# jgsimard/big-dreamer

Hardware: AMD Instinct MI355X
Metric: latent transitions/sec (RSSM + imagination) at batch=50 chunk=50 H=15 (higher is better)
Workload: dtype f32

## Files before the change

big_dreamer_amd/csrc/observe_ksplit.hip:

```cpp
#include "bd_cluster.h"

namespace bd {

#ifdef BD_STAMPS
__device__ unsigned long long g_kstamps[64];
#define BD_KSTAMP(slot)                                                                                  \
    do {                                                                                                 \
        if (blockIdx.x == 0 && threadIdx.x == 0 && t == 5) g_kstamps[slot] = __builtin_amdgcn_s_memtime(); \
    } while (0)
#else
#define BD_KSTAMP(slot)
#endif

constexpr int kKsMaxS = 4;
constexpr int kKsMaxA = 2;

__device__ __forceinline__ void ks_store4(float* p, floatx4 v) {
    asm volatile("s_nop 7\n\ts_nop 3\n\tglobal_store_dwordx4 %0, %1, off sc1\n\ts_nop 1" ::"v"(p), "v"(v) : "memory");
}
__device__ __forceinline__ floatx4 ks_load4(const float* p) {
    const unsigned long long lo = ld_sc1_u64(p), hi = ld_sc1_u64(p + 2);
    return floatx4{__uint_as_float((unsigned)lo), __uint_as_float((unsigned)(lo >> 32)), __uint_as_float((unsigned)hi),
                   __uint_as_float((unsigned)(hi >> 32))};
}

__device__ __forceinline__ void ks_emit(float* img, int lane, floatx4 v) { ks_store4(img + lane * 4, v); }

constexpr int kKsChunk = 8;

__device__ __forceinline__ floatx4 ks_reduce(const float* base, size_t src_stride, int first, int stride, int C, int lane) {
    floatx4 s = floatx4{0.f, 0.f, 0.f, 0.f};
    const float* p = base + lane * 4;
    for (int m0 = first; m0 < C; m0 += kKsChunk * stride) {
        floatx4 v[kKsChunk];
#pragma unroll
        for (int i = 0; i < kKsChunk; ++i) {
            const int src = m0 + i * stride;
            v[i] = floatx4{0.f, 0.f, 0.f, 0.f};
            if (src < C) v[i] = ks_load4(p + (size_t)src * src_stride);
        }
#pragma unroll
        for (int i = 0; i < kKsChunk; ++i) s += v[i];
    }
    return s;
}
__device__ __forceinline__ void ks_handoff(unsigned* flags, int c, int C, unsigned epoch, unsigned* err, unsigned limit,
                                           unsigned code) {
    publish(flags + c, epoch);
    wait_all(flags, C, epoch, err, limit, code);
}
__device__ __forceinline__ floatx4 mfma4(floatx4 a, floatx4 b, floatx4 acc) {
#pragma unroll
    for (int j = 0; j < 4; ++j) acc = mfma16(a[j], b[j], acc);
    return acc;
}
__device__ __forceinline__ void ks_settle(floatx4& v) { asm volatile("" : "+v"(v)); }
template <int N>
__device__ __forceinline__ void ks_settle(floatx4 (&v)[N]) {
#pragma unroll
    for (int i = 0; i < N; ++i) ks_settle(v[i]);
}
#define KS_SETTLE_BEGIN() asm volatile("s_waitcnt vmcnt(0)" ::: "memory")

__device__ __forceinline__ floatx4 ks_frag(const float* w, int nb, int Kb, int kb, int lane, bool ok) {
    return ok ? reinterpret_cast<const floatx4*>(w)[((size_t)nb * Kb + kb) * 64 + lane] : floatx4{0.f, 0.f, 0.f, 0.f};
}

__device__ __forceinline__ floatx4 mfmaT(floatx4 w, floatx4 x, floatx4 acc) {
#pragma unroll
    for (int j = 0; j < 4; ++j) acc = mfma16(w[j], x[j], acc);
    return acc;
}
__device__ __forceinline__ floatx4 ks_row4(const float* p, int n_valid) {
    floatx4 v = floatx4{0.f, 0.f, 0.f, 0.f};
    if (n_valid >= 4) {
        __builtin_memcpy(&v, p, 16);
        return v;
    }
#pragma unroll
    for (int i = 0; i < 4; ++i)
        if (i < n_valid) v[i] = p[i];
    return v;
}
__device__ __forceinline__ void ks_put4(float* p, floatx4 v, int n_valid) {
    if (n_valid >= 4) {
        __builtin_memcpy(p, &v, 16);
        return;
    }
#pragma unroll
    for (int i = 0; i < 4; ++i)
        if (i < n_valid) p[i] = v[i];
}

__global__ __launch_bounds__(kThreads) void observe_kfwd_ns_kernel(bd_observe_fwd_args a_, float* __restrict__ ws, int C, int tiles,
                                                                   unsigned spin_limit) {
    extern __shared__ __attribute__((aligned(16))) float smem[];
    BD_KARGS(bd_observe_fwd_args, ap);
#define a (*ap)
    const ScanDims d(a.Be, a.S, a.A, a.Hd);
    const int Kb_h = d.Kb_h, Kb_s = d.Kb_s, Kb_a = d.Kb_a, Kb_hd = d.Kb_hd;
    const int tile = blockIdx.x / C, c = blockIdx.x - tile * C;
    const int row0 = tile * 16, F = a.Be + a.S, Np = Kb_s * 16;
    const int lane = threadIdx.x & 63;
    const int wave = __builtin_amdgcn_readfirstlane((int)(threadIdx.x >> 6));
    const KsplitFwdLds L(d, a.S);
    float* sf = smem + L.sf;
    float* af = smem + L.af;
    float* red = smem + L.red;
    float* plain = smem + L.plain;
    float* xf = smem + L.xf;
    float* hf = smem + L.hf;
    float* gpart = smem + L.gpart;

    unsigned* flags = reinterpret_cast<unsigned*>(ws) + tile * kMaxCluster;
    unsigned* err = reinterpret_cast<unsigned*>(ws) + tiles * kMaxCluster;
    const KsBuf kb_(C);
    float* xbase = ws + cluster_ws_header_floats(tiles) + (size_t)tile * kKsCopies * kb_.total;

    floatx4 we_s[2][kKsMaxS], we_a[2][kKsMaxA], be4x[2];
    floatx4 wg[2][6], wq[2];
#pragma unroll
    for (int i = 0; i < 2; ++i) {
        const int nbo = wave + kWaves * i;
        const bool ok = nbo < Kb_h;
#pragma unroll
        for (int kb = 0; kb < kKsMaxS; ++kb) we_s[i][kb] = ks_frag(a.w_embed_s, nbo, Kb_s, kb, lane, ok && kb < Kb_s);
#pragma unroll
        for (int kb = 0; kb < kKsMaxA; ++kb) we_a[i][kb] = ks_frag(a.w_embed_a, nbo, Kb_a, kb, lane, ok && kb < Kb_a);
#pragma unroll
        for (int j = 0; j < 4; ++j) {
            const int col = nbo * 16 + 4 * (lane >> 4) + j;
            be4x[i][j] = (ok && col < a.Be) ? a.b_embed[col] : 0.f;
        }
        wg[i][0] = ks_frag(a.w_ir, c, Kb_h, nbo, lane, ok); wg[i][1] = ks_frag(a.w_iz, c, Kb_h, nbo, lane, ok);
        wg[i][2] = ks_frag(a.w_in, c, Kb_h, nbo, lane, ok); wg[i][3] = ks_frag(a.w_hr, c, Kb_h, nbo, lane, ok);
        wg[i][4] = ks_frag(a.w_hz, c, Kb_h, nbo, lane, ok); wg[i][5] = ks_frag(a.w_hn, c, Kb_h, nbo, lane, ok);
        wq[i] = ks_frag(a.w_q1h, nbo, Kb_h, c, lane, nbo < Kb_hd);
    }
    const int npairs = 2 * Kb_s, nparts = kWaves / npairs;
    const int pair = wave % npairs, part = wave / npairs;
    const int pair_nb = pair >> 1, pair_raw = pair & 1;
    const bool has_pair = part == 0, sums_pair = part < nparts;
    floatx4 wh = ks_frag(pair_raw ? a.w_q2s : a.w_q2m, pair_nb, Kb_hd, c, lane, has_pair && c < Kb_hd);
    const int frow = lane & 15, fcol0 = c * 16 + 4 * (lane >> 4);
    const int grow = row0 + frow;
    const int nbe = a.Be - fcol0 < 0 ? 0 : (a.Be - fcol0 < 4 ? a.Be - fcol0 : 4);
    const int nhd = a.Hd - fcol0 < 0 ? 0 : (a.Hd - fcol0 < 4 ? a.Hd - fcol0 : 4);
    const bool rok = grow < a.B;
    floatx4 br4 = floatx4{0.f, 0.f, 0.f, 0.f}, bz4 = br4, bni4 = br4, bnh4 = br4, bq4 = br4;
#pragma unroll
    for (int i = 0; i < 4; ++i) {
        if (i < nbe) {
            const int col = fcol0 + i;
            br4[i] = a.b_ih[col] + a.b_hh[col];
            bz4[i] = a.b_ih[a.Be + col] + a.b_hh[a.Be + col];
            bni4[i] = a.b_ih[2 * a.Be + col];
            bnh4[i] = a.b_hh[2 * a.Be + col];
        }
        if (i < nhd) bq4[i] = a.b_q1[fcol0 + i];
    }
    floatx4 bh4 = floatx4{0.f, 0.f, 0.f, 0.f};
    if (has_pair) {
#pragma unroll
        for (int i = 0; i < 4; ++i) {
            const int col = pair_nb * 16 + 4 * (lane >> 4) + i;
            if (col < a.S) bh4[i] = a.b_q2[pair_raw * a.S + col];
        }
    }
    floatx4 h4 = rok ? ks_row4(a.init_belief + (size_t)grow * a.Be + fcol0, nbe) : floatx4{0.f, 0.f, 0.f, 0.f};
    floatx4* __restrict__ XF4 = reinterpret_cast<floatx4*>(xf);
    floatx4* __restrict__ HF4 = reinterpret_cast<floatx4*>(hf);
#pragma unroll
    for (int i = 0; i < 2; ++i) {
        const int nbo = wave + kWaves * i;
        if (nbo < Kb_h) {
            const int col0 = nbo * 16 + 4 * (lane >> 4);
            const int nv = a.Be - col0 < 0 ? 0 : (a.Be - col0 < 4 ? a.Be - col0 : 4);
            HF4[nbo * 64 + lane] = rok ? ks_row4(a.init_belief + (size_t)grow * a.Be + col0, nv) : floatx4{0.f, 0.f, 0.f, 0.f};
        }
    }
    for (int i = threadIdx.x; i < 16 * Kb_s * 16; i += blockDim.x) {
        const int r = i / (Kb_s * 16), k = i - r * (Kb_s * 16);
        float v = 0.f;
        if (row0 + r < a.B && k < a.S) {
            v = a.init_state[(size_t)(row0 + r) * a.S + k] * (a.nonterm ? a.nonterm[row0 + r] : 1.f);
            if (c == 0 && a.sv_s) a.sv_s[(size_t)(row0 + r) * a.S + k] = v;
        }
        sf[frag_idx(r, k)] = v;
    }
    for (int i = threadIdx.x; i < 16 * Kb_a * 16; i += blockDim.x) {
        const int r = i / (Kb_a * 16), k = i - r * (Kb_a * 16);
        af[frag_idx(r, k)] = (row0 + r < a.B && k < a.A) ? a.actions[(size_t)(row0 + r) * a.A + k] : 0.f;
    }
    lds_barrier();

    KS_SETTLE_BEGIN();
    ks_settle(we_s[0]); ks_settle(we_s[1]); ks_settle(we_a[0]); ks_settle(we_a[1]); ks_settle(be4x);
    ks_settle(wg[0]); ks_settle(wg[1]); ks_settle(wq);
    ks_settle(wh);
    ks_settle(br4); ks_settle(bz4); ks_settle(bni4); ks_settle(bnh4); ks_settle(bq4); ks_settle(bh4); ks_settle(h4);
    const bool lead = (c == 0);
    floatx4* __restrict__ RED4 = reinterpret_cast<floatx4*>(red);
    floatx4* __restrict__ REDB = RED4 + kWaves * 64;
    floatx4* __restrict__ GP4 = reinterpret_cast<floatx4*>(gpart);
    const floatx4 z4 = floatx4{0.f, 0.f, 0.f, 0.f};

    auto load_nt = [&](int t, int e) {
        const int r = e / a.S;
        return (a.nonterm && t < a.T && e < 16 * a.S && row0 + r < a.B) ? a.nonterm[(size_t)t * a.B + row0 + r] : 1.f;
    };
    auto load_ac = [&](int t, int i) {
        const int r = i / (Kb_a * 16), k = i - r * (Kb_a * 16);
        return (t < a.T && i < 16 * Kb_a * 16 && row0 + r < a.B && k < a.A) ? a.actions[((size_t)t * a.B + row0 + r) * a.A + k] : 0.f;
    };

    for (int t = 0; t < a.T; ++t) {
        const size_t tb = (size_t)t * a.B;
        const int tid = bd_tid();
        float* xb = xbase + (size_t)(t & 1) * kb_.total;
        float* hx = xb + kb_.g;
        BD_KSTAMP(0);
        BD_KARGS_FRESH(ap);
        BD_KSTAMP(1);
        {
            const floatx4* __restrict__ S4 = reinterpret_cast<const floatx4*>(sf) + lane;
            const floatx4* __restrict__ A4 = reinterpret_cast<const floatx4*>(af) + lane;
#pragma unroll
            for (int i = 0; i < 2; ++i) {
                const int nbo = wave + kWaves * i;
                if (nbo < Kb_h) {
                    floatx4 acc = be4x[i];
#pragma unroll
                    for (int kb = 0; kb < kKsMaxS; ++kb)
                        if (kb < Kb_s) acc = mfmaT(we_s[i][kb], S4[kb * 64], acc);
#pragma unroll
                    for (int kb = 0; kb < kKsMaxA; ++kb)
                        if (kb < Kb_a) acc = mfmaT(we_a[i][kb], A4[kb * 64], acc);
                    floatx4 x4;
                    const int col0 = nbo * 16 + 4 * (lane >> 4);
#pragma unroll
                    for (int j = 0; j < 4; ++j) x4[j] = (rok && col0 + j < a.Be) ? elu(acc[j]) : 0.f;
                    XF4[nbo * 64 + lane] = x4;
                    if (nbo == c && rok && a.sv_x) ks_put4(a.sv_x + (tb + grow) * a.Be + fcol0, x4, nbe);
                }
            }
        }
        lds_barrier();
        BD_KSTAMP(2);
        BD_KARGS_FRESH(ap);
        {
            floatx4 R = z4, Z = z4, NI = z4, NH = z4;
#pragma unroll
            for (int i = 0; i < 2; ++i) {
                const int kb = wave + kWaves * i;
                if (kb < Kb_h) {
                    const floatx4 xk = XF4[kb * 64 + lane], hk = HF4[kb * 64 + lane];
                    R = mfmaT(wg[i][0], xk, R); Z = mfmaT(wg[i][1], xk, Z); NI = mfmaT(wg[i][2], xk, NI);
                    R = mfmaT(wg[i][3], hk, R); Z = mfmaT(wg[i][4], hk, Z); NH = mfmaT(wg[i][5], hk, NH);
                }
            }
            GP4[(wave * 4 + 0) * 64 + lane] = R; GP4[(wave * 4 + 1) * 64 + lane] = Z;
            GP4[(wave * 4 + 2) * 64 + lane] = NI; GP4[(wave * 4 + 3) * 64 + lane] = NH;
        }
        lds_barrier();
        BD_KSTAMP(3);
        BD_KSTAMP(4);
        {
            const int g = wave & 3, half = wave >> 2;
            floatx4 s4 = z4;
#pragma unroll
            for (int w = 0; w < 4; ++w) s4 += GP4[((half * 4 + w) * 4 + g) * 64 + lane];
            RED4[wave * 64 + lane] = s4;
        }
        lds_barrier();
        {
            const floatx4 R = RED4[0 * 64 + lane] + RED4[4 * 64 + lane] + br4, Z = RED4[1 * 64 + lane] + RED4[5 * 64 + lane] + bz4;
            const floatx4 NI = RED4[2 * 64 + lane] + RED4[6 * 64 + lane] + bni4, NH = RED4[3 * 64 + lane] + RED4[7 * 64 + lane] + bnh4;
            floatx4 rr4, zz4, nn4;
#pragma unroll
            for (int i = 0; i < 4; ++i) {
                rr4[i] = sigmoidf(R[i]);
                zz4[i] = sigmoidf(Z[i]);
                nn4[i] = tanh_act(NI[i] + rr4[i] * NH[i]);
                h4[i] = (rok && i < nbe) ? (1.f - zz4[i]) * nn4[i] + zz4[i] * h4[i] : 0.f;
            }
            if (wave == 0) {
                ks_store4(hx + (size_t)c * 256 + lane * 4, h4);
                if (rok) {
                    ks_put4(a.feat + (tb + grow) * F + fcol0, h4, nbe);
                    if (a.sv_gates) {
                        float* gg = a.sv_gates + (tb + grow) * 4 * a.Be + fcol0;
                        ks_put4(gg, rr4, nbe); ks_put4(gg + a.Be, zz4, nbe); ks_put4(gg + 2 * a.Be, nn4, nbe); ks_put4(gg + 3 * a.Be, NH, nbe);
                    }
                }
            }
        }
        BD_KSTAMP(5);
        BD_KARGS_FRESH(ap);
        const float n_nt = load_nt(t + 1, tid), n_ac = load_ac(t + 1, tid);
        const floatx4 pre4 = rok ? ks_row4(a.pre_emb + (tb + grow) * a.Hd + fcol0, nhd) : z4;
        float eps = 0.f;
        {
            const int row = tid / a.S, col = tid - row * a.S;
            if (tid < 16 * a.S && row0 + row < a.B) eps = a.eps_post[(tb + row0 + row) * a.S + col];
        }
#pragma unroll
        for (int i = 0; i < 2; ++i) {
            const int nbo = wave + kWaves * i;
            if (nbo < Kb_hd) ks_emit(xb + kb_.q + (size_t)(nbo * C + c) * kKsImg, lane, mfmaT(wq[i], h4, z4));
        }
        BD_KSTAMP(6);
        ks_handoff(flags, c, C, (unsigned)(3 * t + 2), err, spin_limit, kErrFwd);
        BD_KSTAMP(7);
        REDB[wave * 64 + lane] = c < Kb_hd ? ks_reduce(xb + kb_.q + (size_t)(c * C) * kKsImg, kKsImg, wave, kWaves, C, lane) : z4;
#pragma unroll
        for (int i = 0; i < 2; ++i) {
            const int nbo = wave + kWaves * i;
            if (nbo < Kb_h) HF4[nbo * 64 + lane] = ks_load4(hx + (size_t)nbo * 256 + lane * 4);
        }
        lds_barrier();
        floatx4 q4 = bq4 + pre4;
        for (int w = 0; w < kWaves; ++w) q4 += REDB[w * 64 + lane];
#pragma unroll
        for (int i = 0; i < 4; ++i) q4[i] = (rok && i < nhd) ? elu(q4[i]) : 0.f;
        if (wave == 0 && rok && a.sv_q) ks_put4(a.sv_q + (tb + grow) * a.Hd + fcol0, q4, nhd);
        BD_KSTAMP(8);
        BD_KARGS_FRESH(ap);
        if (has_pair) ks_emit(xb + kb_.s + (size_t)(c * 8 + pair) * kKsImg, lane, mfmaT(wh, q4, z4));
        BD_KSTAMP(9);
        ks_handoff(flags, c, C, (unsigned)(3 * t + 3), err, spin_limit, kErrFwd);
        BD_KSTAMP(10);
        BD_KARGS_FRESH(ap);
        if (sums_pair) {
            floatx4 v = ks_reduce(xb + kb_.s + (size_t)pair * kKsImg, (size_t)8 * kKsImg, part, nparts, C, lane);
            if (part == 0) v += bh4;
            float* pl = plain + (size_t)part * 2 * 16 * Np;
#pragma unroll
            for (int i = 0; i < 4; ++i) pl[pair_raw * 16 * Np + frow * Np + pair_nb * 16 + 4 * (lane >> 4) + i] = v[i];
        }
        lds_barrier();
        if (tid < 16 * a.S) {
            const int e = tid;
            const int row = e / a.S, col = e - row * a.S;
            const int gr = row0 + row;
            float st = 0.f;
            if (gr < a.B) {
                float Mn = plain[row * Np + col], Rw = plain[16 * Np + row * Np + col];
                for (int pt = 1; pt < nparts; ++pt) {
                    Mn += plain[pt * 2 * 16 * Np + row * Np + col];
                    Rw += plain[pt * 2 * 16 * Np + 16 * Np + row * Np + col];
                }
                const float ee = eps;
                const float sd = softplusf(Rw) + a.min_std;
                st = Mn + sd * ee;
                if (lead) {
                    const size_t ix = (tb + gr) * a.S + col;
                    a.post_mean[ix] = Mn;
                    a.post_std[ix] = sd;
                    a.feat[(tb + gr) * F + a.Be + col] = st;
                }
            }
            const float mv = st * n_nt;
            sf[frag_idx(row, col)] = mv;
            if (lead && a.sv_s && t + 1 < a.T && gr < a.B) a.sv_s[(tb + a.B + gr) * a.S + col] = mv;
        }
        if (tid < 16 * Kb_a * 16) af[frag_idx(tid / (Kb_a * 16), tid % (Kb_a * 16))] = n_ac;
        lds_barrier();
        BD_KSTAMP(11);
    }
#undef a
}

__global__ __launch_bounds__(kThreads) void observe_kbwd_kernel(bd_observe_bwd_args a_, float* __restrict__ ws, int C, int tiles,
                                                                unsigned spin_limit) {
    extern __shared__ __attribute__((aligned(16))) float smem[];
    BD_KARGS(bd_observe_bwd_args, ap);
#define a (*ap)
    const ScanDims d(a.Be, a.S, a.A, a.Hd);
    const int Kb_h = d.Kb_h, Kb_s = d.Kb_s, Kb_hd = d.Kb_hd;
    const int tile = blockIdx.x / C, c = blockIdx.x - tile * C;
    const int row0 = tile * 16, F = a.Be + a.S;
    const int lane = threadIdx.x & 63;
    const int wave = __builtin_amdgcn_readfirstlane((int)(threadIdx.x >> 6));
    const KsplitBwdLds L(d, a.S);
    float* dM = smem + L.dM;
    float* dRaw = smem + L.dRaw;
    float* ds_plain = smem + L.ds_plain;
    const int nparts = L.nparts;
    const int dsp_stride = L.dsp_stride;
    float* red = smem + L.red;

    unsigned* flags = reinterpret_cast<unsigned*>(ws) + tile * kMaxCluster;
    unsigned* err = reinterpret_cast<unsigned*>(ws) + tiles * kMaxCluster;
    const KsBuf kb_(C);
    float* xbase = ws + cluster_ws_header_floats(tiles) + (size_t)tile * kKsCopies * kb_.total;

    floatx4 w2m[kKsMaxS], w2s[kKsMaxS];
#pragma unroll
    for (int kb = 0; kb < kKsMaxS; ++kb) {
        w2m[kb] = ks_frag(a.wt_q2m, c, Kb_s, kb, lane, kb < Kb_s && c < Kb_hd);
        w2s[kb] = ks_frag(a.wt_q2s, c, Kb_s, kb, lane, kb < Kb_s && c < Kb_hd);
    }
    floatx4 w1[2], wg[2][6];
#pragma unroll
    for (int i = 0; i < 2; ++i) {
        const int nbo = wave + kWaves * i;
        const bool ok = nbo < Kb_h;
        w1[i] = ks_frag(a.wt_q1h, nbo, Kb_hd, c, lane, ok && c < Kb_hd);
        wg[i][0] = ks_frag(a.wt_ir, nbo, Kb_h, c, lane, ok); wg[i][1] = ks_frag(a.wt_iz, nbo, Kb_h, c, lane, ok);
        wg[i][2] = ks_frag(a.wt_in, nbo, Kb_h, c, lane, ok); wg[i][3] = ks_frag(a.wt_hr, nbo, Kb_h, c, lane, ok);
        wg[i][4] = ks_frag(a.wt_hz, nbo, Kb_h, c, lane, ok); wg[i][5] = ks_frag(a.wt_hn, nbo, Kb_h, c, lane, ok);
    }
    const int sblk = wave % Kb_s, spart = wave / Kb_s;
    floatx4 wes = ks_frag(a.wt_embed_s, sblk, Kb_h, c, lane, spart == 0);
    const int frow = lane & 15, fcol0 = c * 16 + 4 * (lane >> 4);
    const int grow = row0 + frow;
    const int nbe = a.Be - fcol0 < 0 ? 0 : (a.Be - fcol0 < 4 ? a.Be - fcol0 : 4);
    const int nhd = a.Hd - fcol0 < 0 ? 0 : (a.Hd - fcol0 < 4 ? a.Hd - fcol0 : 4);
    const bool rok = grow < a.B;

    for (int i = threadIdx.x; i < nparts * dsp_stride; i += blockDim.x) ds_plain[i] = 0.f;
    lds_barrier();

    KS_SETTLE_BEGIN();
    ks_settle(w2m); ks_settle(w2s); ks_settle(w1); ks_settle(wg[0]); ks_settle(wg[1]);
    ks_settle(wes);
    const bool lead = (c == 0);
    floatx4* __restrict__ RED4 = reinterpret_cast<floatx4*>(red);
    floatx4* __restrict__ REDB = RED4 + kWaves * 64;
    const floatx4 z4 = floatx4{0.f, 0.f, 0.f, 0.f};
    floatx4 dhc4 = z4;
    unsigned epoch = 0;

    struct B1v { float dfs, dpm, eps, dps, pstd; };
    struct Svv { floatx4 svq4, svx4, gr4, gz4, gn4, gh4, hp4, dft4; };
    auto load_b1 = [&](int t, int i) {
        B1v v{0.f, 0.f, 0.f, 0.f, 0.f};
        const int r = i / (Kb_s * 16), k = i - r * (Kb_s * 16);
        const int gr = row0 + r;
        if (i < 16 * Kb_s * 16 && gr < a.B && k < a.S) {
            const size_t tb = (size_t)t * a.B, idx = (tb + gr) * a.S + k;
            v.dfs = a.dfeat[(tb + gr) * F + a.Be + k];
            v.dpm = a.dpost_mean ? a.dpost_mean[idx] : 0.f;
            v.eps = a.eps_post[idx];
            v.dps = a.dpost_std ? a.dpost_std[idx] : 0.f;
            v.pstd = a.post_std[idx];
        }
        return v;
    };
    auto load_sv = [&](int t) {
        Svv v;
        v.svq4 = floatx4{1.f, 1.f, 1.f, 1.f};
        v.svx4 = v.svq4;
        v.gr4 = v.gz4 = v.gn4 = v.gh4 = v.hp4 = v.dft4 = z4;
        if (rok) {
            const size_t tb = (size_t)t * a.B;
            v.svq4 = ks_row4(a.sv_q + (tb + grow) * a.Hd + fcol0, nhd);
            v.svx4 = ks_row4(a.sv_x + (tb + grow) * a.Be + fcol0, nbe);
            const float* gg = a.sv_gates + (tb + grow) * 4 * a.Be + fcol0;
            v.gr4 = ks_row4(gg, nbe); v.gz4 = ks_row4(gg + a.Be, nbe); v.gn4 = ks_row4(gg + 2 * a.Be, nbe); v.gh4 = ks_row4(gg + 3 * a.Be, nbe);
            v.hp4 = t > 0 ? ks_row4(a.feat + (tb - a.B + grow) * F + fcol0, nbe) : ks_row4(a.init_belief + (size_t)grow * a.Be + fcol0, nbe);
            v.dft4 = ks_row4(a.dfeat + (tb + grow) * F + fcol0, nbe);
        }
        return v;
    };
    B1v nb1{0.f, 0.f, 0.f, 0.f, 0.f};
    Svv nsv{z4, z4, z4, z4, z4, z4, z4, z4};
    nb1 = load_b1(a.T - 1, (int)threadIdx.x);
    nsv = load_sv(a.T - 1);

    for (int t = a.T - 1; t >= 0; --t) {
        const size_t tb = (size_t)t * a.B;
        const int tid = bd_tid();
        float* xb = xbase + (size_t)(t & 1) * kb_.total;
        BD_KSTAMP(16);
        BD_KARGS_FRESH(ap);
        const B1v cb1 = nb1;
        const Svv sv = nsv;
        if (t > 0) {
            nb1 = load_b1(t - 1, tid);
            nsv = load_sv(t - 1);
        }
        if (tid < 16 * Kb_s * 16) {
            const int i = tid;
            const int r = i / (Kb_s * 16), k = i - r * (Kb_s * 16);
            const int gr = row0 + r;
            float dm = 0.f, dr = 0.f;
            if (gr < a.B && k < a.S) {
                const B1v v = cb1;
                float dst = v.dfs;
                for (int pt = 0; pt < nparts; ++pt) dst += ds_plain[pt * dsp_stride + r * a.S + k];
                dm = dst + v.dpm;
                const float dsd = dst * v.eps + v.dps;
                dr = dsd * one_minus_exp_neg(v.pstd - a.min_std);
                if (lead) {
                    a.d_q2_out[(tb + gr) * 2 * a.S + k] = dm;
                    a.d_q2_out[(tb + gr) * 2 * a.S + a.S + k] = dr;
                }
            }
            dM[frag_idx(r, k)] = dm;
            dRaw[frag_idx(r, k)] = dr;
        }
        const floatx4 svq4 = sv.svq4, svx4 = sv.svx4, gr4 = sv.gr4, gz4 = sv.gz4, gn4 = sv.gn4, gh4 = sv.gh4, hp4 = sv.hp4, dft4 = sv.dft4;
        lds_barrier();
        BD_KSTAMP(17);
        floatx4 dq4;
        {
            floatx4 acc = z4;
            const floatx4* __restrict__ M4 = reinterpret_cast<const floatx4*>(dM) + lane;
            const floatx4* __restrict__ R4 = reinterpret_cast<const floatx4*>(dRaw) + lane;
#pragma unroll
            for (int kb = 0; kb < kKsMaxS; ++kb)
                if (kb < Kb_s) {
                    acc = mfmaT(w2m[kb], M4[kb * 64], acc);
                    acc = mfmaT(w2s[kb], R4[kb * 64], acc);
                }
#pragma unroll
            for (int i = 0; i < 4; ++i) dq4[i] = (rok && i < nhd) ? acc[i] * elu_grad_from_out(svq4[i]) : 0.f;
            if (wave == 0 && rok) ks_put4(a.d_q1_pre + (tb + grow) * a.Hd + fcol0, dq4, nhd);
        }
        BD_KSTAMP(18);
        BD_KARGS_FRESH(ap);
        ++epoch;
#pragma unroll
        for (int i = 0; i < 2; ++i) {
            const int nbo = wave + kWaves * i;
            if (nbo < Kb_h) ks_emit(xb + kb_.q + (size_t)(nbo * C + c) * kKsImg, lane, mfmaT(w1[i], dq4, z4));
        }
        BD_KSTAMP(19);
        ks_handoff(flags, c, C, epoch, err, spin_limit, kErrBwd);
        BD_KSTAMP(20);
        RED4[wave * 64 + lane] = ks_reduce(xb + kb_.q + (size_t)(c * C) * kKsImg, kKsImg, wave, kWaves, C, lane);
        lds_barrier();
        floatx4 vr4, vz4, vni4, vnh4, carry4;
        {
            floatx4 dh4 = dhc4 + dft4;
            for (int w = 0; w < kWaves; ++w) dh4 += RED4[w * 64 + lane];
#pragma unroll
            for (int i = 0; i < 4; ++i) {
                const bool ok = rok && i < nbe;
                const float dh = ok ? dh4[i] : 0.f;
                const float rr = gr4[i], zz = gz4[i], nn = gn4[i], hn = gh4[i];
                const float dn = dh * (1.f - zz);
                const float dz = dh * (hp4[i] - nn);
                vni4[i] = dn * (1.f - nn * nn);
                vnh4[i] = vni4[i] * rr;
                vr4[i] = vni4[i] * hn * rr * (1.f - rr);
                vz4[i] = dz * zz * (1.f - zz);
                carry4[i] = dh * zz;
            }
            if (wave == 0 && rok) {
                float* gi = a.d_gi + (tb + grow) * 3 * a.Be + fcol0;
                float* ghh = a.d_gh + (tb + grow) * 3 * a.Be + fcol0;
                ks_put4(gi, vr4, nbe); ks_put4(gi + a.Be, vz4, nbe); ks_put4(gi + 2 * a.Be, vni4, nbe);
                ks_put4(ghh, vr4, nbe); ks_put4(ghh + a.Be, vz4, nbe); ks_put4(ghh + 2 * a.Be, vnh4, nbe);
            }
        }
        BD_KSTAMP(21);
        BD_KARGS_FRESH(ap);
        ++epoch;
#pragma unroll
        for (int i = 0; i < 2; ++i) {
            const int nbo = wave + kWaves * i;
            if (nbo < Kb_h) {
                floatx4 DX = mfmaT(wg[i][0], vr4, z4), DH = mfmaT(wg[i][3], vr4, z4);
                DX = mfmaT(wg[i][1], vz4, DX); DH = mfmaT(wg[i][4], vz4, DH);
                DX = mfmaT(wg[i][2], vni4, DX); DH = mfmaT(wg[i][5], vnh4, DH);
                float* dst = xb + kb_.g + ((size_t)(nbo * C + c) * 2) * kKsImg;
                ks_emit(dst, lane, DX); ks_emit(dst + kKsImg, lane, DH);
            }
        }
        BD_KSTAMP(22);
        ks_handoff(flags, c, C, epoch, err, spin_limit, kErrBwd);
        BD_KSTAMP(23);
        {
            const int g = wave & 1, quarter = wave >> 1;
            REDB[wave * 64 + lane] = ks_reduce(xb + kb_.g + ((size_t)(c * C) * 2 + g) * kKsImg, (size_t)2 * kKsImg, quarter, 4, C, lane);
        }
        lds_barrier();
        floatx4 de4;
        {
            floatx4 DX = z4, DH = z4;
            for (int qd = 0; qd < 4; ++qd) { DX += REDB[(2 * qd) * 64 + lane]; DH += REDB[(2 * qd + 1) * 64 + lane]; }
#pragma unroll
            for (int i = 0; i < 4; ++i) {
                const bool ok = rok && i < nbe;
                de4[i] = ok ? DX[i] * elu_grad_from_out(svx4[i]) : 0.f;
                dhc4[i] = ok ? carry4[i] + DH[i] : 0.f;
            }
            if (wave == 0 && rok) ks_put4(a.d_embed_pre + (tb + grow) * a.Be + fcol0, de4, nbe);
        }
        BD_KSTAMP(24);
        BD_KARGS_FRESH(ap);
        ++epoch;
        if (spart == 0) ks_emit(xb + kb_.s + (size_t)(c * 8 + sblk) * kKsImg, lane, mfmaT(wes, de4, z4));
        BD_KSTAMP(25);
        ks_handoff(flags, c, C, epoch, err, spin_limit, kErrBwd);
        BD_KSTAMP(26);
        BD_KARGS_FRESH(ap);
        if (spart < nparts) {
            const floatx4 v = ks_reduce(xb + kb_.s + (size_t)sblk * kKsImg, (size_t)8 * kKsImg, spart, nparts, C, lane);
            const float mk = rok ? (a.nonterm ? a.nonterm[tb + grow] : 1.f) : 0.f;
#pragma unroll
            for (int i = 0; i < 4; ++i) {
                const int col = sblk * 16 + 4 * (lane >> 4) + i;
                if (col < a.S) ds_plain[spart * dsp_stride + frow * a.S + col] = v[i] * mk;
            }
        }
        lds_barrier();
        BD_KSTAMP(27);
    }
#undef a
}

int& ksplit_mode() {
    static int m = -1;
    return m;
}

bool ksplit_ok(int Be, int S, int A, int Hd, int C) {
    if (ksplit_mode() == 0) return false;
    return C == cdiv(Be, 16) && C <= 2 * kWaves && cdiv(Hd, 16) <= C && cdiv(S, 16) <= kKsMaxS && cdiv(A, 16) <= kKsMaxA &&
           S <= kHeadMaxN && 16 * S <= kThreads && 2 * cdiv(S, 16) <= kWaves;
}

static int ks_reset(float* ws, int tiles, hipStream_t stream, const char* who) {
    if (hipMemsetAsync(ws, 0, cluster_ws_flag_floats(tiles) * sizeof(float), stream) != hipSuccess) return fail("%s: memset failed", who);
    return 0;
}

int launch_observe_kfwd(const bd_observe_fwd_args* a, float* ws, int C, int tiles, hipStream_t stream) {
    if (allow_big_lds(observe_kfwd_ns_kernel)) return -1;
    const KsplitFwdLds L(ScanDims(a->Be, a->S, a->A, a->Hd), a->S);
    BD_REQUIRE(L.vec_ok(), "bd_observe_forward_cluster: misaligned LDS layout");
    const size_t dyn = launch_lds(observe_kfwd_ns_kernel, (size_t)L.total * sizeof(float), "bd_observe_forward_cluster");
    if (!dyn) return -1;
    if (ks_reset(ws, tiles, stream, "bd_observe_forward_cluster")) return -1;
    hipLaunchKernelGGL(observe_kfwd_ns_kernel, dim3(tiles * C), dim3(kThreads), dyn, stream, *a, ws, C, tiles, cluster_spin_limit());
    BD_CHECK_LAUNCH("bd_observe_forward_cluster");
    return 0;
}
int launch_observe_kbwd(const bd_observe_bwd_args* a, float* ws, int C, int tiles, hipStream_t stream) {
    if (allow_big_lds(observe_kbwd_kernel)) return -1;
    const KsplitBwdLds L(ScanDims(a->Be, a->S, a->A, a->Hd), a->S);
    BD_REQUIRE(L.vec_ok(), "bd_observe_backward_cluster: misaligned LDS layout");
    const size_t dyn = launch_lds(observe_kbwd_kernel, (size_t)L.total * sizeof(float), "bd_observe_backward_cluster");
    if (!dyn) return -1;
    if (ks_reset(ws, tiles, stream, "bd_observe_backward_cluster")) return -1;
    hipLaunchKernelGGL(observe_kbwd_kernel, dim3(tiles * C), dim3(kThreads), dyn, stream, *a, ws, C, tiles, cluster_spin_limit());
    BD_CHECK_LAUNCH("bd_observe_backward_cluster");
    return 0;
}

}

#ifdef BD_STAMPS
extern "C" int bd_debug_kstamps(unsigned long long* out64) {
    return hipMemcpyFromSymbol(out64, HIP_SYMBOL(bd::g_kstamps), sizeof(unsigned long long) * 64) == hipSuccess ? 0 : -1;
}
#endif
```

Before: 13.94 million.

## Overlap cross-block barrier spins with prefetch loads and hidden-state MFMAs

Replaces the publish-then-wait handoff with a wait routine that runs work pieces while the first wave polls the flags. In the forward pass, next-step loads are issued during the first barrier. The h-dependent gate MFMAs and the action-embedding MFMAs for the next step are computed during the second barrier. In the backward pass, next-step prefetch loads move into the barrier wait, and address computation is simplified with precomputed offsets and a vector-aligned fast path. This aims to hide inter-block synchronization latency, at the cost of more live registers and more intricate ordering; the af update also moves earlier in the step.

```diff
diff --git a/big_dreamer_amd/csrc/observe_ksplit.hip b/big_dreamer_amd/csrc/observe_ksplit.hip
--- a/big_dreamer_amd/csrc/observe_ksplit.hip
+++ b/big_dreamer_amd/csrc/observe_ksplit.hip
@@ -48,6 +48,48 @@
                                            unsigned code) {
     publish(flags + c, epoch);
     wait_all(flags, C, epoch, err, limit, code);
+}
+template <int K>
+struct ks_ix { static constexpr int value = K; };
+template <class Piece>
+__device__ __forceinline__ void ks_wait_all_work(const unsigned* flags, int C, unsigned epoch, unsigned* err, unsigned limit,
+                                                 unsigned code, Piece piece) {
+    if ((threadIdx.x >> 6) == 0) {
+        const int lane = threadIdx.x & 63;
+        unsigned spins = 0;
+        const unsigned* fl = flags + (lane < C ? lane : 0);
+        auto issue = [&] { return __hip_atomic_load(fl, __ATOMIC_RELAXED, __HIP_MEMORY_SCOPE_AGENT); };
+        auto landed = [&](unsigned v) {
+            asm volatile("" : "+v"(v));
+            return lane < C ? v : epoch;
+        };
+        auto passed = [&](unsigned v) {
+            if (__all(v >= epoch)) return true;
+            if (++spins > limit) {
+                if (lane == 0) __hip_atomic_fetch_or(err, code, __ATOMIC_RELAXED, __HIP_MEMORY_SCOPE_AGENT);
+                return true;
+            }
+            return false;
+        };
+        unsigned v = issue();
+        piece(ks_ix<0>{});
+        bool done = passed(landed(v));
+        if (!done) {
+            v = issue();
+            piece(ks_ix<1>{});
+            done = passed(landed(v));
+        } else {
+            piece(ks_ix<1>{});
+        }
+        while (!done) {
+            __builtin_amdgcn_s_sleep(2);
+            done = passed(landed(issue()));
+        }
+    } else {
+        piece(ks_ix<0>{});
+        piece(ks_ix<1>{});
+    }
+    lds_barrier();
 }
 __device__ __forceinline__ floatx4 mfma4(floatx4 a, floatx4 b, floatx4 acc) {
 #pragma unroll
@@ -205,6 +247,25 @@
     floatx4* __restrict__ GP4 = reinterpret_cast<floatx4*>(gpart);
     const floatx4 z4 = floatx4{0.f, 0.f, 0.f, 0.f};
 
+    floatx4 hR = z4, hZ = z4, hN = z4, xa0 = z4, xa1 = z4;
+    auto ahead = [&](auto ix) __attribute__((always_inline)) {
+        constexpr int i = decltype(ix)::value;
+        const int kb = wave + kWaves * i;
+        if constexpr (i == 0) hR = hZ = hN = z4;
+        if (kb < Kb_h) {
+            const floatx4 hk = HF4[kb * 64 + lane];
+            hR = mfmaT(wg[i][3], hk, hR); hZ = mfmaT(wg[i][4], hk, hZ); hN = mfmaT(wg[i][5], hk, hN);
+            const floatx4* __restrict__ A4 = reinterpret_cast<const floatx4*>(af) + lane;
+            floatx4 acc = be4x[i];
+#pragma unroll
+            for (int k = 0; k < kKsMaxA; ++k)
+                if (k < Kb_a) acc = mfmaT(we_a[i][k], A4[k * 64], acc);
+            if constexpr (i == 0) xa0 = acc; else xa1 = acc;
+        }
+    };
+    ahead(ks_ix<0>{});
+    ahead(ks_ix<1>{});
+
     auto load_nt = [&](int t, int e) {
         const int r = e / a.S;
         return (a.nonterm && t < a.T && e < 16 * a.S && row0 + r < a.B) ? a.nonterm[(size_t)t * a.B + row0 + r] : 1.f;
@@ -224,18 +285,15 @@
         BD_KSTAMP(1);
         {
             const floatx4* __restrict__ S4 = reinterpret_cast<const floatx4*>(sf) + lane;
-            const floatx4* __restrict__ A4 = reinterpret_cast<const floatx4*>(af) + lane;
 #pragma unroll
             for (int i = 0; i < 2; ++i) {
                 const int nbo = wave + kWaves * i;
                 if (nbo < Kb_h) {
-                    floatx4 acc = be4x[i];
+                    floatx4 acc = xa0;
+                    if (i) acc = xa1;
 #pragma unroll
                     for (int kb = 0; kb < kKsMaxS; ++kb)
                         if (kb < Kb_s) acc = mfmaT(we_s[i][kb], S4[kb * 64], acc);
-#pragma unroll
-                    for (int kb = 0; kb < kKsMaxA; ++kb)
-                        if (kb < Kb_a) acc = mfmaT(we_a[i][kb], A4[kb * 64], acc);
                     floatx4 x4;
                     const int col0 = nbo * 16 + 4 * (lane >> 4);
 #pragma unroll
@@ -249,18 +307,17 @@
         BD_KSTAMP(2);
         BD_KARGS_FRESH(ap);
         {
-            floatx4 R = z4, Z = z4, NI = z4, NH = z4;
+            floatx4 R = hR, Z = hZ, NI = z4;
 #pragma unroll
             for (int i = 0; i < 2; ++i) {
                 const int kb = wave + kWaves * i;
                 if (kb < Kb_h) {
-                    const floatx4 xk = XF4[kb * 64 + lane], hk = HF4[kb * 64 + lane];
+                    const floatx4 xk = XF4[kb * 64 + lane];
                     R = mfmaT(wg[i][0], xk, R); Z = mfmaT(wg[i][1], xk, Z); NI = mfmaT(wg[i][2], xk, NI);
-                    R = mfmaT(wg[i][3], hk, R); Z = mfmaT(wg[i][4], hk, Z); NH = mfmaT(wg[i][5], hk, NH);
                 }
             }
             GP4[(wave * 4 + 0) * 64 + lane] = R; GP4[(wave * 4 + 1) * 64 + lane] = Z;
-            GP4[(wave * 4 + 2) * 64 + lane] = NI; GP4[(wave * 4 + 3) * 64 + lane] = NH;
+            GP4[(wave * 4 + 2) * 64 + lane] = NI; GP4[(wave * 4 + 3) * 64 + lane] = hN;
         }
         lds_barrier();
         BD_KSTAMP(3);
@@ -297,20 +354,24 @@
         }
         BD_KSTAMP(5);
         BD_KARGS_FRESH(ap);
-        const float n_nt = load_nt(t + 1, tid), n_ac = load_ac(t + 1, tid);
-        const floatx4 pre4 = rok ? ks_row4(a.pre_emb + (tb + grow) * a.Hd + fcol0, nhd) : z4;
-        float eps = 0.f;
-        {
-            const int row = tid / a.S, col = tid - row * a.S;
-            if (tid < 16 * a.S && row0 + row < a.B) eps = a.eps_post[(tb + row0 + row) * a.S + col];
-        }
 #pragma unroll
         for (int i = 0; i < 2; ++i) {
             const int nbo = wave + kWaves * i;
             if (nbo < Kb_hd) ks_emit(xb + kb_.q + (size_t)(nbo * C + c) * kKsImg, lane, mfmaT(wq[i], h4, z4));
         }
         BD_KSTAMP(6);
-        ks_handoff(flags, c, C, (unsigned)(3 * t + 2), err, spin_limit, kErrFwd);
+        float n_nt = 1.f, n_ac = 0.f, eps = 0.f;
+        floatx4 pre4 = z4;
+        publish(flags + c, (unsigned)(3 * t + 2));
+        ks_wait_all_work(flags, C, (unsigned)(3 * t + 2), err, spin_limit, kErrFwd, [&](auto ix) __attribute__((always_inline)) {
+            if constexpr (decltype(ix)::value == 0) {
+                n_nt = load_nt(t + 1, tid);
+                n_ac = load_ac(t + 1, tid);
+                if (rok) pre4 = ks_row4(a.pre_emb + (tb + grow) * a.Hd + fcol0, nhd);
+                const int row = tid / a.S, col = tid - row * a.S;
+                if (tid < 16 * a.S && row0 + row < a.B) eps = a.eps_post[(tb + row0 + row) * a.S + col];
+            }
+        });
         BD_KSTAMP(7);
         REDB[wave * 64 + lane] = c < Kb_hd ? ks_reduce(xb + kb_.q + (size_t)(c * C) * kKsImg, kKsImg, wave, kWaves, C, lane) : z4;
 #pragma unroll
@@ -318,6 +379,7 @@
             const int nbo = wave + kWaves * i;
             if (nbo < Kb_h) HF4[nbo * 64 + lane] = ks_load4(hx + (size_t)nbo * 256 + lane * 4);
         }
+        if (tid < 16 * Kb_a * 16) af[frag_idx(tid / (Kb_a * 16), tid % (Kb_a * 16))] = n_ac;
         lds_barrier();
         floatx4 q4 = bq4 + pre4;
         for (int w = 0; w < kWaves; ++w) q4 += REDB[w * 64 + lane];
@@ -328,7 +390,8 @@
         BD_KARGS_FRESH(ap);
         if (has_pair) ks_emit(xb + kb_.s + (size_t)(c * 8 + pair) * kKsImg, lane, mfmaT(wh, q4, z4));
         BD_KSTAMP(9);
-        ks_handoff(flags, c, C, (unsigned)(3 * t + 3), err, spin_limit, kErrFwd);
+        publish(flags + c, (unsigned)(3 * t + 3));
+        ks_wait_all_work(flags, C, (unsigned)(3 * t + 3), err, spin_limit, kErrFwd, ahead);
         BD_KSTAMP(10);
         BD_KARGS_FRESH(ap);
         if (sums_pair) {
@@ -364,7 +427,6 @@
             sf[frag_idx(row, col)] = mv;
             if (lead && a.sv_s && t + 1 < a.T && gr < a.B) a.sv_s[(tb + a.B + gr) * a.S + col] = mv;
         }
-        if (tid < 16 * Kb_a * 16) af[frag_idx(tid / (Kb_a * 16), tid % (Kb_a * 16))] = n_ac;
         lds_barrier();
         BD_KSTAMP(11);
     }
@@ -434,39 +496,62 @@
 
     struct B1v { float dfs, dpm, eps, dps, pstd; };
     struct Svv { floatx4 svq4, svx4, gr4, gz4, gn4, gh4, hp4, dft4; };
-    auto load_b1 = [&](int t, int i) {
+    int b1_s = -1, b1_f = 0;
+    {
+        const int i = threadIdx.x, r = i / (Kb_s * 16), k = i - r * (Kb_s * 16);
+        if (i < 16 * Kb_s * 16 && row0 + r < a.B && k < a.S) {
+            b1_s = (row0 + r) * a.S + k;
+            b1_f = (row0 + r) * F + a.Be + k;
+        }
+    }
+    const int o_hd = grow * a.Hd + fcol0, o_be = grow * a.Be + fcol0, o_g = grow * 4 * a.Be + fcol0, o_f = grow * F + fcol0;
+    auto load_b1 = [&](int t) __attribute__((always_inline)) {
         B1v v{0.f, 0.f, 0.f, 0.f, 0.f};
-        const int r = i / (Kb_s * 16), k = i - r * (Kb_s * 16);
-        const int gr = row0 + r;
-        if (i < 16 * Kb_s * 16 && gr < a.B && k < a.S) {
-            const size_t tb = (size_t)t * a.B, idx = (tb + gr) * a.S + k;
-            v.dfs = a.dfeat[(tb + gr) * F + a.Be + k];
-            v.dpm = a.dpost_mean ? a.dpost_mean[idx] : 0.f;
-            v.eps = a.eps_post[idx];
-            v.dps = a.dpost_std ? a.dpost_std[idx] : 0.f;
-            v.pstd = a.post_std[idx];
+        const float *dfeat = a.dfeat, *dpm = a.dpost_mean, *eps = a.eps_post, *dps = a.dpost_std, *pstd = a.post_std;
+        asm volatile("" ::"s"(dfeat), "s"(dpm), "s"(eps), "s"(dps), "s"(pstd));
+        if (b1_s >= 0) {
+            const size_t tb = (size_t)t * a.B, idx = tb * a.S + b1_s;
+            v.dfs = dfeat[tb * F + b1_f];
+            v.dpm = dpm ? dpm[idx] : 0.f;
+            v.eps = eps[idx];
+            v.dps = dps ? dps[idx] : 0.f;
+            v.pstd = pstd[idx];
         }
         return v;
     };
-    auto load_sv = [&](int t) {
+    auto load_sv = [&](int t) __attribute__((always_inline)) {
         Svv v;
         v.svq4 = floatx4{1.f, 1.f, 1.f, 1.f};
         v.svx4 = v.svq4;
         v.gr4 = v.gz4 = v.gn4 = v.gh4 = v.hp4 = v.dft4 = z4;
+        const float *sv_q = a.sv_q, *sv_x = a.sv_x, *sv_g = a.sv_gates, *dfeat = a.dfeat;
+        const float* hprev = t > 0 ? a.feat + (size_t)(t - 1) * a.B * F + o_f : a.init_belief + o_be;
+        asm volatile("" ::"s"(sv_q), "s"(sv_x), "s"(sv_g), "s"(dfeat));
         if (rok) {
             const size_t tb = (size_t)t * a.B;
-            v.svq4 = ks_row4(a.sv_q + (tb + grow) * a.Hd + fcol0, nhd);
-            v.svx4 = ks_row4(a.sv_x + (tb + grow) * a.Be + fcol0, nbe);
-            const float* gg = a.sv_gates + (tb + grow) * 4 * a.Be + fcol0;
-            v.gr4 = ks_row4(gg, nbe); v.gz4 = ks_row4(gg + a.Be, nbe); v.gn4 = ks_row4(gg + 2 * a.Be, nbe); v.gh4 = ks_row4(gg + 3 * a.Be, nbe);
-            v.hp4 = t > 0 ? ks_row4(a.feat + (tb - a.B + grow) * F + fcol0, nbe) : ks_row4(a.init_belief + (size_t)grow * a.Be + fcol0, nbe);
-            v.dft4 = ks_row4(a.dfeat + (tb + grow) * F + fcol0, nbe);
+            const float *pq = sv_q + tb * a.Hd + o_hd, *px = sv_x + tb * a.Be + o_be, *gg = sv_g + tb * 4 * a.Be + o_g;
+            const float* pd = dfeat + tb * F + o_f;
+            if ((nbe & 3) == 0 && (nhd & 3) == 0) {
+                if (nhd) v.svq4 = ks_row4(pq, 4);
+                if (nbe) {
+                    v.svx4 = ks_row4(px, 4);
+                    v.gr4 = ks_row4(gg, 4); v.gz4 = ks_row4(gg + a.Be, 4); v.gn4 = ks_row4(gg + 2 * a.Be, 4); v.gh4 = ks_row4(gg + 3 * a.Be, 4);
+                    v.hp4 = ks_row4(hprev, 4);
+                    v.dft4 = ks_row4(pd, 4);
+                }
+            } else {
+                v.svq4 = ks_row4(pq, nhd);
+                v.svx4 = ks_row4(px, nbe);
+                v.gr4 = ks_row4(gg, nbe); v.gz4 = ks_row4(gg + a.Be, nbe); v.gn4 = ks_row4(gg + 2 * a.Be, nbe); v.gh4 = ks_row4(gg + 3 * a.Be, nbe);
+                v.hp4 = ks_row4(hprev, nbe);
+                v.dft4 = ks_row4(pd, nbe);
+            }
         }
         return v;
     };
     B1v nb1{0.f, 0.f, 0.f, 0.f, 0.f};
     Svv nsv{z4, z4, z4, z4, z4, z4, z4, z4};
-    nb1 = load_b1(a.T - 1, (int)threadIdx.x);
+    nb1 = load_b1(a.T - 1);
     nsv = load_sv(a.T - 1);
 
     for (int t = a.T - 1; t >= 0; --t) {
@@ -477,10 +562,6 @@
         BD_KARGS_FRESH(ap);
         const B1v cb1 = nb1;
         const Svv sv = nsv;
-        if (t > 0) {
-            nb1 = load_b1(t - 1, tid);
-            nsv = load_sv(t - 1);
-        }
         if (tid < 16 * Kb_s * 16) {
             const int i = tid;
             const int r = i / (Kb_s * 16), k = i - r * (Kb_s * 16);
@@ -595,7 +676,15 @@
         ++epoch;
         if (spart == 0) ks_emit(xb + kb_.s + (size_t)(c * 8 + sblk) * kKsImg, lane, mfmaT(wes, de4, z4));
         BD_KSTAMP(25);
-        ks_handoff(flags, c, C, epoch, err, spin_limit, kErrBwd);
+        publish(flags + c, epoch);
+        ks_wait_all_work(flags, C, epoch, err, spin_limit, kErrBwd, [&](auto ix) __attribute__((always_inline)) {
+            if constexpr (decltype(ix)::value == 0) {
+                if (t > 0) {
+                    nb1 = load_b1(t - 1);
+                    nsv = load_sv(t - 1);
+                }
+            }
+        });
         BD_KSTAMP(26);
         BD_KARGS_FRESH(ap);
         if (spart < nparts) {
```

Result: no change. 14.03 million, median of 6 (+0.6%).
